# tiangexiang/OccNeRF

Hardware: AMD Instinct MI355X
Metric: rays/sec at 512x512x128spp, random-init ckpt (higher is better)
Workload: dtype f32; 1 GPU; BASELINE configs[1]: free-view frame, 512x512 image, 128 samples/ray, non-rigid motion on, seeded random-init checkpoint; synthetic SMPL-like body and camera; 183784 rays hit the body bbox (ray_mask); H2D of the ray batch and the prior and D2H of [R,5] inside the step; the frame's rays sharded over the ranks; samples whose motion-weight sum is exactly 0 are dropped after the warp (bit-identical pi; rays_per_frame=183784, samples_per_ray=128, skip_empty_samples=True, dedup_repeated_samples=False, knn_center_cache=True, warp_bone_culling=True, world_size_formed=1

## Files before the change

include/occnerf_hip.h:

```cpp
#ifndef OCCNERF_HIP_H
#define OCCNERF_HIP_H

#include <stdint.h>

#ifdef __cplusplus
extern "C" {
#endif

#define OCCNERF_ABI_VERSION 5

int occnerf_abi_version(void);
const char *occnerf_last_error(void);

int occnerf_experiment_knob(const char *name, int value);


int occnerf_grid_encode_forward(const float *inputs, const float *embeddings,
                                const int32_t *offsets, float *outputs, uint32_t B, uint32_t D,
                                uint32_t C, uint32_t L, float S, uint32_t H, float *dy_dx,
                                uint32_t gridtype, int align_corners, uint32_t interp,
                                void *stream);

int occnerf_grid_encode_backward(const float *grad, const float *inputs, const float *embeddings,
                                 const int32_t *offsets, float *grad_embeddings, uint32_t B,
// ... 289 lines not shown
                         const double *h_dist, int32_t win_y, int32_t win_x, int32_t win_h, int32_t win_w,
                         uint8_t *out_image, uint8_t *out_mask, void *stream);

int occnerf_resize_frame(const uint8_t *image, const uint8_t *mask, int32_t H, int32_t W, int32_t h, int32_t w,
                         const int32_t *x_off_lanczos, const float *x_w_lanczos, const int32_t *y_off_lanczos,
                         const float *y_w_lanczos, const int32_t *x_off_bilinear, const float *x_w_bilinear,
                         const int32_t *y_off_bilinear, const float *y_w_bilinear, const int32_t *h_x_off_lanczos,
                         const int32_t *h_y_off_lanczos, const int32_t *h_x_off_bilinear, const int32_t *h_y_off_bilinear,
                         const float *h_bgcolor, double *img64, double *alpha64, void *stream);

int occnerf_patch_batch_f64(const double *img64, const double *alpha64, const float *rays8, const uint8_t *box_mask,
                            int32_t H, int32_t W, int32_t n_patches, int32_t size, const double *h_u, double subject_ratio,
                            const float *h_bgcolor, int32_t *row_counts, float *rays, float *near, float *far,
                            float *target_rgbs, float *target_patches, uint8_t *patch_masks, int32_t *patch_div_indices,
                            int32_t *xy_min, int32_t *pix_of_row, int32_t *row_of_pix, int32_t *n_rows, void *stream);
int occnerf_whole_frame_gather_f64(const double *img64, const double *alpha64, const float *rays8, const uint8_t *box_mask,
                                   int32_t H, int32_t W, const float *h_bgcolor, const int32_t *row_start, int32_t R,
                                   int64_t *ray_index, float *rays, float *near, float *far, float *target_rgbs,
                                   double *ray_alpha, uint8_t *truth_u8, float *gt_vis, float *gt_alpha, void *stream);

#define OCCNERF_FRAME_METRICS_RECORD 14
int64_t occnerf_frame_metrics_workspace_bytes(int32_t N, int32_t H, int32_t W);
int occnerf_frame_metrics(const uint8_t *pred, const uint8_t *truth, const float *alpha, const uint8_t *body,
                          const float *gt_vis_alpha, const float *gt_alpha, int32_t N, int32_t H, int32_t W,
                          double data_range, double *record, double *ssim_map, void *workspace, void *stream);

int32_t occnerf_progress_tile_blocks(int32_t height, int32_t width);
int occnerf_progress_tile(const float *rgb, const int64_t *ray_index, int64_t R, int32_t height, int32_t width,
                          const float *h_bgcolor01, const double *h_bgcolor255, const uint8_t *truth_u8, uint8_t *mosaic,
                          int32_t mosaic_rows, int32_t mosaic_cols, int32_t tile_x, int32_t tile_y, int32_t *partial,
                          int32_t *off_bg, void *stream);


int occnerf_mesh_count(const float *field, int32_t nx, int32_t ny, int32_t nz, float level, int32_t *row_count,
                       void *stream);
int occnerf_mesh_emit(const float *field, int32_t nx, int32_t ny, int32_t nz, float level, const int64_t *row_start,
                      int64_t T, int64_t *tri_keys, void *stream);
int occnerf_mesh_vertices(const int64_t *keys, int64_t V, const float *field, int32_t nx, int32_t ny, int32_t nz,
                          float level, const double *h_bbox_min, double h, float *pos, void *stream);

int occnerf_mesh_pose(const float *x_c, int64_t V, const float *Rs, const float *Ts, const float *vol, int32_t nb, int32_t G,
                      const float *h_bbox_min, const float *h_bbox_scale, int32_t candidates, int32_t max_iter, double tol,
                      float *p_out, uint8_t *flag, uint8_t *iters, float *resid, void *stream);


int occnerf_mesh_project(const float *pos, int64_t V, const double *h_K, const double *h_E, int32_t *xy, double *z,
                         uint8_t *vflag, void *stream);
int occnerf_mesh_raster(const int32_t *faces, int64_t T, int64_t V, const int32_t *xy, const double *z, const uint8_t *vflag,
                        int32_t H, int32_t W, uint64_t *keys, int32_t *wide_list, int32_t *counts, void *stream);
int occnerf_mesh_resolve(const uint64_t *keys, const int32_t *faces, int64_t T, int64_t V, const int32_t *xy, const double *z,
                         const uint8_t *vflag, const uint8_t *colors, const uint8_t *h_bgcolor, int32_t H, int32_t W,
                         uint8_t *cover, int32_t *tri, float *depth, uint8_t *rgb, int32_t *counts, void *stream);

#ifdef __cplusplus
}
#endif
#endif
```

occnerf_amd/_lib.py:

```python
import ctypes as C
import os

_HERE = os.path.dirname(os.path.abspath(__file__))
LIB_PATH = os.environ.get('OCCNERF_HIP_LIB') or os.path.join(_HERE, 'liboccnerf_hip.so')

ABI_VERSION = 5

_vp, _i32, _i64, _u32, _f32 = C.c_void_p, C.c_int32, C.c_int64, C.c_uint32, C.c_float

SIGNATURES = {
    'occnerf_abi_version': (C.c_int, []),
    'occnerf_last_error': (C.c_char_p, []),
    'occnerf_experiment_knob': (C.c_int, [C.c_char_p, C.c_int]),
    'occnerf_grid_encode_forward': (C.c_int, [_vp, _vp, _vp, _vp, _u32, _u32, _u32, _u32, _f32, _u32,
                                               _vp, _u32, C.c_int, _u32, _vp]),
    'occnerf_grid_encode_backward': (C.c_int, [_vp, _vp, _vp, _vp, _vp, _u32, _u32, _u32, _u32, _f32,
                                                _u32, _vp, _vp, _u32, C.c_int, _u32, _vp]),
    'occnerf_grid_grad_runs': (C.c_int, [_vp, _vp, _i64, _u32, _u32, _u32, _vp, _vp]),
    'occnerf_grid_encode_forward_h': (C.c_int, [_vp, _vp, _vp, _vp, _vp, _u32, _u32, _u32, _u32, _f32, _u32,
                                                 _vp, _u32, C.c_int, _u32, _vp]),
    'occnerf_grid_encode_backward_h': (C.c_int, [_vp, _vp, _vp, _vp, _vp, _vp, _u32, _u32, _u32, _u32, _f32,
                                                  _u32, _vp, _vp, _u32, C.c_int, _u32, _vp, _i64, _vp]),
    'occnerf_grid_encode_forward_f16': (C.c_int, [_vp, _vp, _vp, _vp, _u32, _u32, _u32, _u32, _f32, _u32,
                                                   _vp, _u32, C.c_int, _u32, _vp]),
# ... 67 lines not shown
    'occnerf_canonical_mlp_bf16x3': (C.c_int, [_vp, _i64, _vp, _vp, _vp, _i32, _vp]),
    'occnerf_canonical_mlp_pack_f16': (C.c_int, [_vp, _vp, _vp]),
    'occnerf_canonical_mlp_f16x3': (C.c_int, [_vp, _vp, _i64, _vp, _vp, _vp, _vp, _vp, _vp]),
    'occnerf_nonrigid_pack_f16': (C.c_int, [_vp, _vp, _vp]),
    'occnerf_nonrigid_f16x3': (C.c_int, [_vp, _i64, _vp, _vp, _vp, _vp, _vp, _vp, _vp, _vp, _vp, _vp, _vp]),
    'occnerf_canonical_mlp_bf16x3_rows': (C.c_int, [_vp, _vp, _i64, _vp, _vp, _vp, _vp, _i32, _vp]),
    'occnerf_composite': (C.c_int, [_vp, _vp, _vp, _vp, _vp, _i64, _i32, _vp, _vp, _vp, _vp, _vp, _vp, _vp]),
    'occnerf_linear_pack': (C.c_int, [_vp, _vp, _i32, _i32, _vp, _i32, _vp, _i32, _i32, _vp, _vp, _vp, _vp]),
    'occnerf_linear_forward': (C.c_int, [_vp, _i64, _i32, _vp, _i64, _i32, _vp, _vp, _i32, _vp, _i64, _vp, _i64, _i32,
                                          _i32, _vp, _i32, _i64, _i64, _i32, _i32, _vp]),
    'occnerf_linear_wgrad_slices': (_i32, [_i64]),
    'occnerf_linear_wgrad': (C.c_int, [_vp, _i64, _i32, _vp, _i64, _i32, _i64, _i32, _vp, _vp, _vp]),
    'occnerf_linear_wgrad_reduce': (C.c_int, [_vp, _vp, _i32, _i32, _i32, _vp, _vp, _vp, _i32, _vp, _i32, _vp]),
    'occnerf_composite_backward': (C.c_int, [_vp, _vp, _vp, _vp, _vp, _i64, _i32, _vp, _vp, _vp, _vp, _vp, _vp]),
    'occnerf_warp_backward_slices': (_i32, [_i64]),
    'occnerf_warp_backward': (C.c_int, [_vp, _i64, _i32, _vp, _vp, _vp, _vp, _vp, _i32, _i32, _vp, _vp, _vp, _vp, _vp]),
    'occnerf_agg_weights': (C.c_int, [_vp, _vp, _i64, _i32, _vp, _vp, _vp]),
    'occnerf_pose_motion_bases': (C.c_int, [_vp, _vp, _vp, _i32, _vp, _vp, _vp, _vp, _vp, _vp]),
    'occnerf_pose_motion_bases_backward': (C.c_int, [_vp, _vp, _vp, _vp, _vp, _vp, _vp, _vp, _vp, _vp, _vp]),
    'occnerf_prior_softmax': (C.c_int, [_vp, _vp, _i32, _i64, _vp, _vp]),
    'occnerf_pack_rays': (C.c_int, [_vp, _vp, _vp, _vp, _i64, _vp, _vp]),
    'occnerf_assemble_image': (C.c_int, [_vp, _vp, _vp, _i64, _i32, _i32, _vp, _vp, _vp, _vp]),
    'occnerf_convt3d_col2im': (C.c_int, [_vp, _vp, _i32, _i32, _i32, _i32, _vp, _vp]),
    'occnerf_convt3d_im2col': (C.c_int, [_vp, _i32, _i32, _i32, _i32, _vp, _vp]),
    'occnerf_adam_table_row_bytes': (_i32, []),
    'occnerf_adam_step': (C.c_int, [_vp, _i32, _vp, _i32, _i32] + [C.c_double] * 4 + [_vp, _vp]),
    'occnerf_lpips_packed_floats': (_i64, []),
    'occnerf_lpips_workspace_floats': (_i64, [_i32, _i32, _i32]),
    'occnerf_lpips_pack': (C.c_int, [_vp, _vp, _vp, _vp, _vp, _vp, _vp]),
    'occnerf_lpips_forward': (C.c_int, [_vp, _vp, _vp, _i32, _i32, _i32, _i32, _vp, _vp, _vp, _vp]),
    'occnerf_lpips_backward': (C.c_int, [_vp, _vp, _i32, _i32, _i32, _i32, _vp, _vp, _vp, _vp]),
    'occnerf_patch_assemble': (C.c_int, [_vp, _vp, _i64, _i32, _i32, _vp, _vp, _vp]),
    'occnerf_patch_assemble_backward': (C.c_int, [_vp, _vp, _i64, _vp, _vp]),
    'occnerf_patch_batch_max_patches': (_i32, []),
    'occnerf_patch_batch': (C.c_int, [_vp, _vp, _vp, _vp, _i32, _i32, _i32, _i32, _vp, C.c_double, _vp] + [_vp] * 12 + [_vp]),
    'occnerf_whole_frame_count': (C.c_int, [_vp, _i32, _i32, _vp, _vp]),
    'occnerf_whole_frame_gather': (C.c_int, [_vp, _vp, _vp, _vp, _i32, _i32, _vp, _vp, _i32] + [_vp] * 9 + [_vp]),
    'occnerf_view_frame_gather': (C.c_int, [_vp, _vp, _i32, _i32, _vp, _i32, _vp, _vp, _vp, _vp, _vp]),
    'occnerf_undistort_u8': (C.c_int, [_vp, _vp, _i32, _i32, _vp, _vp, _i32, _i32, _i32, _i32, _vp, _vp, _vp]),
    'occnerf_resize_frame': (C.c_int, [_vp, _vp, _i32, _i32, _i32, _i32] + [_vp] * 8 + [_vp] * 4 + [_vp, _vp, _vp, _vp]),
    'occnerf_patch_batch_f64': (C.c_int, [_vp, _vp, _vp, _vp, _i32, _i32, _i32, _i32, _vp, C.c_double, _vp] + [_vp] * 12 + [_vp]),
    'occnerf_whole_frame_gather_f64': (C.c_int, [_vp, _vp, _vp, _vp, _i32, _i32, _vp, _vp, _i32] + [_vp] * 9 + [_vp]),
    'occnerf_frame_metrics_workspace_bytes': (_i64, [_i32, _i32, _i32]),
    'occnerf_frame_metrics': (C.c_int, [_vp, _vp, _vp, _vp, _vp, _vp, _i32, _i32, _i32, C.c_double, _vp, _vp, _vp, _vp]),
    'occnerf_progress_tile_blocks': (_i32, [_i32, _i32]),
    'occnerf_progress_tile': (C.c_int, [_vp, _vp, _i64, _i32, _i32, _vp, _vp, _vp, _vp, _i32, _i32, _i32, _i32, _vp, _vp, _vp]),
    'occnerf_mesh_count': (C.c_int, [_vp, _i32, _i32, _i32, _f32, _vp, _vp]),
    'occnerf_mesh_emit': (C.c_int, [_vp, _i32, _i32, _i32, _f32, _vp, _i64, _vp, _vp]),
    'occnerf_mesh_vertices': (C.c_int, [_vp, _i64, _vp, _i32, _i32, _i32, _f32, _vp, C.c_double, _vp, _vp]),
    'occnerf_mesh_pose': (C.c_int, [_vp, _i64, _vp, _vp, _vp, _i32, _i32, _vp, _vp, _i32, _i32, C.c_double, _vp, _vp, _vp, _vp, _vp]),
    'occnerf_mesh_project': (C.c_int, [_vp, _i64, _vp, _vp, _vp, _vp, _vp, _vp]),
    'occnerf_mesh_raster': (C.c_int, [_vp, _i64, _i64, _vp, _vp, _vp, _i32, _i32, _vp, _vp, _vp, _vp]),
    'occnerf_mesh_resolve': (C.c_int, [_vp, _vp, _i64, _i64, _vp, _vp, _vp, _vp, _vp, _i32, _i32, _vp, _vp, _vp, _vp, _vp, _vp]),
}

_lib = None


def lib():
    global _lib
    if _lib is None:
        if not os.path.exists(LIB_PATH):
            raise ImportError(
                f'{LIB_PATH} not found: the gfx950 kernels are not built. Run '
                '`python -c "import __graft_entry__ as g; g.build()"` (or `make -C '
                'occnerf_amd/csrc`). There is no CPU fallback for this path.')
        import torch
        handle = C.CDLL(LIB_PATH)
        for name, (res, args) in SIGNATURES.items():
            fn = getattr(handle, name)
            fn.restype, fn.argtypes = res, args
        if handle.occnerf_abi_version() != ABI_VERSION:
            raise ImportError(f'liboccnerf_hip.so: ABI version {handle.occnerf_abi_version()}, this binding was written '
                              f'for {ABI_VERSION} (include/occnerf_hip.h OCCNERF_ABI_VERSION): rebuild the library')
        _lib = handle
    return _lib


def check(rc, what):
    if rc != 0:
        msg = lib().occnerf_last_error().decode(errors='replace')
        raise RuntimeError(f'{what} failed ({rc}): {msg}')
```

occnerf_amd/csrc/compact.hip:

```cpp
#include "common.h"

#include <hipcub/hipcub.hpp>

namespace occ {

struct LivePredicate {
    const float *mask;
    __device__ bool operator()(const int &i) const { return mask[i] != 0.0f; }
};

__global__ void scatter_raw_kernel(const float *__restrict__ raw_c, const int32_t *__restrict__ rows,
                                   const int32_t *__restrict__ n_dev, float *__restrict__ raw_full) {
    const int64_t m = (int64_t)blockIdx.x * blockDim.x + threadIdx.x;
    if (m >= (int64_t)*n_dev) return;
    const int64_t n = rows[m];
#pragma unroll
    for (int c = 0; c < 5; c++) raw_full[n * 5 + c] = raw_c[m * 5 + c];
}

struct RepeatFlag {
    const uint32_t *keys;
    int64_t stride;
    int K;
    const int32_t *rows;
// ... 240 lines not shown
        hipLaunchKernelGGL(unique_remap_kernel, dim3((unsigned)((scan_cap + 255) / 256)), dim3(256), 0, st, scan, n_scan_dev,
                           rep);
    return check_launch("unique_heads");
}

OCC_API int occnerf_scatter_raw_heads(const float *raw_h, const float *raw_c, const int32_t *rows, const int32_t *n_dev,
                                      const int32_t *scanA, const int32_t *scanB, int64_t N_max, float *raw_full,
                                      void *stream) {
    using namespace occ;
    if (N_max <= 0) return 0;
    OCC_REQUIRE(raw_h && raw_c && rows && n_dev && raw_full, "scatter_raw_heads: null argument");
    const int64_t blocks = (N_max + 255) / 256;
    OCC_REQUIRE(blocks < (1ll << 31), "scatter_raw_heads: N too large");
    hipLaunchKernelGGL(scatter_raw_heads_kernel, dim3((unsigned)blocks), dim3(256), 0, as_stream(stream), raw_h, raw_c,
                       rows, n_dev, scanA, scanB, raw_full);
    return check_launch("scatter_raw_heads");
}

OCC_API int64_t occnerf_live_rows_temp_bytes(int64_t N) {
    using namespace occ;
    if (N <= 0 || N >= (1ll << 31)) return 0;
    size_t bytes = 0;
    hipcub::CountingInputIterator<int> it(0);
    if (hipcub::DeviceSelect::If(nullptr, bytes, it, (int *)nullptr, (int *)nullptr, (int)N, LivePredicate{nullptr},
                                 (hipStream_t)0) != hipSuccess)
        return -1;
    return (int64_t)bytes;
}

OCC_API int occnerf_live_rows(const float *mask, int64_t N, int32_t *rows, int32_t *count, void *temp,
                              int64_t temp_bytes, void *stream) {
    using namespace occ;
    OCC_REQUIRE(mask && rows && count && temp, "live_rows: null argument");
    OCC_REQUIRE(N > 0 && N < (1ll << 31), "live_rows: N=%lld out of range", (long long)N);
    size_t bytes = (size_t)temp_bytes;
    hipcub::CountingInputIterator<int> it(0);
    const hipError_t e = hipcub::DeviceSelect::If(temp, bytes, it, rows, count, (int)N, LivePredicate{mask},
                                                  as_stream(stream));
    OCC_REQUIRE(e == hipSuccess, "live_rows: %s", hipGetErrorString(e));
    return check_launch("live_rows");
}

OCC_API int occnerf_scatter_raw(const float *raw_c, const int32_t *rows, const int32_t *n_dev, int64_t N_max,
                                float *raw_full, void *stream) {
    using namespace occ;
    if (N_max <= 0) return 0;
    OCC_REQUIRE(raw_c && rows && n_dev && raw_full, "scatter_raw: null argument");
    const int64_t blocks = (N_max + 255) / 256;
    OCC_REQUIRE(blocks < (1ll << 31), "scatter_raw: N too large");
    hipLaunchKernelGGL(scatter_raw_kernel, dim3((unsigned)blocks), dim3(256), 0, as_stream(stream), raw_c, rows, n_dev,
                       raw_full);
    return check_launch("scatter_raw");
}
```

occnerf_amd/network.py:

```python
import os

import numpy as np
import torch
import torch.nn as nn

from . import geometry, ops
from .canonical_mlp import CanonicalMLP
from .config import get_cfg
from .rayorder import ray_patch_order
from .modules import (BodyPoseRefiner, MotionBasisComputer, MotionWeightVolumeDecoder,
                      NonRigidMotionMLP, hann_window_weights)


class _Replica(nn.Module):

    def __init__(self, module):
        super().__init__()
        self.module = module

    def forward(self, *a, **k):
        return self.module(*a, **k)


def _load_smpl(cfg):
# ... 175 lines not shown
        dec_mod = self.mweight_vol_decoder
        enc = self.cnl_mlp.module.encoder
        srcs = list(dec_mod.parameters()) + [self.point_dist, self.point_base, enc.embeddings]
        key = tuple((t.data_ptr(), t._version) for t in srcs)
        if self._wconst is not None and self._wconst['key'] == key:
            return self._wconst
        with torch.no_grad():
            dec = dec_mod.decoder.forward_gemm(dec_mod.const_embedding[None])[0].contiguous()
            table = self._point_stage(self._context())
        self._wconst = {'key': key, 'dec': dec, 'table': table}
        return self._wconst

    def _point_pack(self, wc):
        srcs = [self.point_counter, self.point_base]
        key = (wc['table'].data_ptr(),) + tuple((t.data_ptr(), t._version) for t in srcs)
        if wc.get('pack_key') != key:
            ctx = self._context()
            wc['pack'] = ops.point_pack(self.point_base.detach(), ctx['normals'], ctx['unit'],
                                        self.point_counter.detach(), wc['table'])
            wc['pack_key'] = key
        return wc['pack']

    def _point_stage(self, ctx):
        enc = self.cnl_mlp.module.encoder
        pc = self.point_cloud.detach().float().contiguous()
        base = self.point_base.detach()
        kidx = ops.knn_small(pc, base, 3)
        knn_base, sdf = ops.point_sdf(pc, base, ctx['normals'], ctx['unit'], kidx)
        table = ops.point_table(knn_base, sdf, pc, ctx['bound32'], ctx['two_bound32'],
                                enc.embeddings.detach(), enc.offsets, enc.log2_per_level_scale,
                                enc.base_resolution)
        return table

    def _stage_features(self, rays8, z, xyz, mask, pk, cond, hann, table, pack, center=None):
        cfg, ctx = self.cfg, self._context()
        S = int(cfg.N_samples)
        enc = self.cnl_mlp.module.encoder
        rows, count = ops.live_rows(mask)
        self.last_live_count = count
        dedup = bool(cfg.get('dedup_repeated_samples', True))
        scan_a = scan_b = mrows = mcount = None
        frows, fcount, kmask = rows, count, mask
        if not cfg.ignore_non_rigid_motions:
            if pk['nr_bf16'] is not None:
                ops.nonrigid_bf16x3_rows(xyz, rows, count, cond, hann, pk['nr_w0'], pk['nr_b0'], pk['nr'], pk['nr_bf16'],
                                         domain_flag=pk['domain_flag'])
            else:
                ops.nonrigid_rows(xyz, rows, count, cond, hann, pk['nr_w0'], pk['nr_b0'], pk['nr'])
        if dedup:
            scan_a, frows, fcount, kmask = ops.repeat_heads(xyz, 3, count, rows=rows,
                                                            want_mask=not cfg.get('knn_query_list', True))
            if cfg.get('dedup_global_positions', False):
                frows, fcount = ops.unique_heads(xyz, 3, frows, fcount, scan=scan_a, scan_count=count)
        self.last_head_counts = (fcount, None)
        if cfg.get('knn_query_list', True):
            knn = ops.msknn_clustered(xyz, rays8.shape[0], S, ctx['clusters'], ctx['seed'], rows=frows, count=fcount, center=center)
        else:
            knn = ops.msknn_clustered(xyz, rays8.shape[0], S, ctx['clusters'], ctx['seed'], mask=kmask, center=center)
        if center is not None and len(center) > 3 and center[3] != self._center_stamp(table):
            raise RuntimeError('stale kNN centre: its cached feature row was computed from another table / counter / embedding '
                               'version than this frame\'s (ops.sample_features freshness contract)')
        mlp_in, raw_c, _ = ops.sample_features(
            xyz, knn, self.point_base.detach(), ctx['normals'], ctx['unit'],
            self.point_counter.detach(), table, ctx['bound32'], ctx['two_bound32'],
            enc.embeddings.detach(), enc.offsets, enc.log2_per_level_scale, enc.base_resolution,
            rows=frows, count=fcount, pack=pack, center=None if center is None else center[0],
            center_agg=None if center is None else center[2])
        del knn
        if dedup:
            scan_b, mrows, mcount, _ = ops.repeat_heads(mlp_in, 68, fcount)
            if cfg.get('dedup_global', True):
                mrows, mcount = ops.unique_heads(mlp_in, 68, mrows, mcount, scan=scan_b, scan_count=fcount)
            self.last_head_counts = (fcount, mcount)
        return {'dedup': dedup, 'rays8': rays8, 'z': z, 'mask': mask, 'rows': rows, 'count': count, 'mlp_in': mlp_in,
                'raw_c': raw_c, 'scan_a': scan_a, 'scan_b': scan_b, 'mrows': mrows, 'mcount': mcount, 'cnl': pk['cnl'],
                'cnl_bf16': pk['cnl_bf16'], 'domain_flag': pk['domain_flag'], 'N': xyz.shape[0]}

    @staticmethod
    def _stage_mlp_composite(st, bgcolor, out, out_rows):
        dev, N = st['mlp_in'].device, st['N']

        def mlp(raw_out, count, in_rows=None):
            if st['cnl_bf16'] is not None:
                ops.canonical_mlp_bf16x3(st['mlp_in'], st['cnl'], st['cnl_bf16'], raw_out, count=count, in_rows=in_rows,
                                         domain_flag=st['domain_flag'])
            else:
                ops.canonical_mlp(st['mlp_in'], st['cnl'], raw_out, count=count, in_rows=in_rows)
        if st['dedup']:
            raw_h = torch.empty(st['mlp_in'].shape[0], 5, device=dev)
            mlp(raw_h, st['mcount'], st['mrows'])
            raw = ops.scatter_raw_heads(raw_h, st['raw_c'], st['rows'], st['count'], st['scan_a'], st['scan_b'],
                                        torch.zeros(N, 5, device=dev))
        else:
            mlp(st['raw_c'], st['count'])
            raw = ops.scatter_raw(st['raw_c'], st['rows'], st['count'], torch.zeros(N, 5, device=dev))
        st['mlp_in'] = None
        return ops.composite(raw, st['mask'], st['z'], st['rays8'], bgcolor, out=out, out_rows=out_rows)[:3]

    def _nonrigid_f16_pack(self):
        pk = self._packed_weights()
        if pk.get('nr_f16_train') is None:
            nr_lin = [m for m in self.non_rigid_mlp.module.block_mlps if isinstance(m, nn.Linear)]
            pk['nr_f16_train'] = pk['nr_bf16'] if (pk['nr_bf16'] is not None and pk['nr_bf16'].dtype == torch.float16) else \
                ops.nonrigid_pack_f16([m.weight.detach() for m in nr_lin])
        return pk['nr_f16_train']

    def _knn_center_lists(self, cond, hann):
        ctx, pk = self._context(), self._packed_weights()
        c = torch.zeros(64, 3, device=self.point_base.device)
        if not self.cfg.ignore_non_rigid_motions:
            c = ops.nonrigid(c, cond, hann, pk['nr_w0'], pk['nr_b0'], pk['nr'], direct=True)
        return ops.knn_center(c[0].contiguous(), ctx['points'], ctx['index_map'], ctx['scale_begin'])

    def _knn_center(self, cond, hann, table, pack):
        ctx, pk = self._context(), self._packed_weights()
        c = torch.zeros(64, 3, device=self.point_base.device)
        if not self.cfg.ignore_non_rigid_motions:
            c = ops.nonrigid(c, cond, hann, pk['nr_w0'], pk['nr_b0'], pk['nr'], direct=True)
        center, idx = ops.knn_center(c[0].contiguous(), ctx['points'], ctx['index_map'], ctx['scale_begin'])
        enc = self.cnl_mlp.module.encoder
        row, _, enc_in = ops.sample_features(
            c[:8].contiguous(), idx[None].expand(8, -1, -1).contiguous(), self.point_base.detach(), ctx['normals'], ctx['unit'],
            self.point_counter.detach(), table, ctx['bound32'], ctx['two_bound32'], enc.embeddings.detach(), enc.offsets,
            enc.log2_per_level_scale, enc.base_resolution, pack=pack, want_enc_in=True)
        return center, idx, ops.center_row(row[0], enc_in[0]), self._center_stamp(table)

    def _center_stamp(self, table):
        return (table.data_ptr(), table._version, self.point_counter._version, self.cnl_mlp.module.encoder.embeddings._version)

    def _render_rays(self, rays8, Rs, Ts, vol, bbox_min, bbox_scale, bgcolor, cond, hann,
                     table, t_rand=None, out=None, out_rows=None, pack=None, boxes=None, center=None):
        cfg, ctx = self.cfg, self._context()
        S = int(cfg.N_samples)
        enc = self.cnl_mlp.module.encoder
        t_vals = torch.linspace(0., 1., steps=S, device=rays8.device)
        z, xyz, mask, _ = ops.sample_warp(rays8, S, t_vals, Rs, Ts, vol, bbox_min, bbox_scale,
                                          t_rand=t_rand, boxes=boxes)
        pk = self._packed_weights()
        N = xyz.shape[0]
        if cfg.get('skip_empty_samples', True) and cfg.get('knn_culling', True):
            st = self._stage_features(rays8, z, xyz, mask, pk, cond, hann, table, pack, center)
            return self._stage_mlp_composite(st, bgcolor, out, out_rows)

        if not cfg.ignore_non_rigid_motions:
            if pk['nr_bf16'] is not None:
                ops.nonrigid_bf16x3(xyz, cond, hann, pk['nr_w0'], pk['nr_b0'], pk['nr'], pk['nr_bf16'], out=xyz, domain_flag=pk['domain_flag'])
            else:
# ... 264 lines not shown
```

occnerf_amd/ops.py:

```python
import ctypes as C

import numpy as np
import torch

from . import _lib

_f32p = C.POINTER(C.c_float)


def _chk(t, dtype, name):
    if not torch.is_tensor(t):
        raise RuntimeError(f'{name} must be a tensor')
    if not t.is_cuda:
        raise RuntimeError(f'{name} must be a CUDA(HIP) tensor; there is no CPU path')
    if not t.is_contiguous():
        raise RuntimeError(f'{name} must be a contiguous tensor')
    if t.dtype != dtype:
        raise RuntimeError(f'{name} must be {dtype}, got {t.dtype}')
    return t.data_ptr()


def _guard_dev(dev):
    if torch.device(dev).type != 'cuda':
        raise RuntimeError(f'tensors are on {dev}: this path runs on a GPU only, there is no CPU path')
# ... 211 lines not shown
    return packed


def nonrigid(xyz, cond, hann, W0, b0, packed, out=None, direct=False):
    out = torch.empty_like(xyz) if out is None else out
    _kh, ph = _host_f32(hann, 6)
    fn = _lib.lib().occnerf_nonrigid_direct if direct else _lib.lib().occnerf_nonrigid
    with _guard(xyz):
        rc = fn(
            _chk(xyz, torch.float32, 'xyz'), xyz.shape[0], _chk(cond, torch.float32, 'cond'), ph,
            _chk(W0, torch.float32, 'W0'), _chk(b0, torch.float32, 'b0'),
            _chk(packed, torch.float32, 'packed'), _chk(out, torch.float32, 'xyz_out'), _stream(xyz))
    _lib.check(rc, 'nonrigid')
    return out


def nonrigid_rows(xyz, rows, count, cond, hann, W0, b0, packed):
    _kh, ph = _host_f32(hann, 6)
    with _guard(xyz):
        rc = _lib.lib().occnerf_nonrigid_rows(
            _chk(xyz, torch.float32, 'xyz'), rows.shape[0], _chk(rows, torch.int32, 'rows'),
            _chk(count, torch.int32, 'count'), _chk(cond, torch.float32, 'cond'), ph,
            _chk(W0, torch.float32, 'W0'), _chk(b0, torch.float32, 'b0'), _chk(packed, torch.float32, 'packed'),
            _stream(xyz))
    _lib.check(rc, 'nonrigid_rows')
    return xyz


def live_rows(mask):
    N = mask.shape[0]
    dev = mask.device
    nbytes = int(_lib.lib().occnerf_live_rows_temp_bytes(N))
    if nbytes < 0:
        raise RuntimeError('live_rows: temp size query failed')
    temp = torch.empty(max(nbytes, 16), device=dev, dtype=torch.uint8)
    rows = torch.empty(N, device=dev, dtype=torch.int32)
    count = torch.empty(1, device=dev, dtype=torch.int32)
    with _guard(mask):
        rc = _lib.lib().occnerf_live_rows(_chk(mask, torch.float32, 'mask'), N, rows.data_ptr(), count.data_ptr(),
                                          temp.data_ptr(), nbytes, _stream(mask))
    _lib.check(rc, 'live_rows')
    return rows, count


def scatter_raw(raw_c, rows, count, raw_full):
    with _guard(raw_c):
        rc = _lib.lib().occnerf_scatter_raw(_chk(raw_c, torch.float32, 'raw_c'), _chk(rows, torch.int32, 'rows'),
                                            _chk(count, torch.int32, 'count'), rows.shape[0],
                                            _chk(raw_full, torch.float32, 'raw_full'), _stream(raw_c))
    _lib.check(rc, 'scatter_raw')
    return raw_full


def repeat_heads(keys, key_cols, count, rows=None, want_mask=False):
    dev = keys.device
    if keys.dim() != 2 or not keys.is_contiguous() or keys.element_size() != 4:
        raise RuntimeError('repeat_heads: keys must be a contiguous [M, C] tensor of 4-byte elements')
    cap = keys.shape[0] if rows is None else rows.shape[0]
    scan = torch.empty(cap, device=dev, dtype=torch.int32)
    heads = torch.empty(cap, device=dev, dtype=torch.int32)
    head_count = torch.empty(1, device=dev, dtype=torch.int32)
    head_mask = torch.zeros(keys.shape[0], device=dev, dtype=torch.float32) if want_mask else None
    if cap == 0:
        head_count.zero_()
        return scan, heads, head_count, head_mask
    nbytes = int(_lib.lib().occnerf_repeat_heads_temp_bytes(cap))
    if nbytes < 0:
        raise RuntimeError('repeat_heads: temp size query failed')
    temp = torch.empty(max(nbytes, 16), device=dev, dtype=torch.uint8)
    with _guard_dev(dev):
        rc = _lib.lib().occnerf_repeat_heads(
            keys.data_ptr(), keys.shape[1], int(key_cols), _opt(rows, torch.int32, 'rows'),
            _chk(count, torch.int32, 'count'), cap, scan.data_ptr(), heads.data_ptr(), head_count.data_ptr(),
            None if head_mask is None else head_mask.data_ptr(), temp.data_ptr(), nbytes, _stream(keys))
    _lib.check(rc, 'repeat_heads')
    return scan, heads, head_count, head_mask


def unique_heads(keys, key_cols, heads, count, scan=None, scan_count=None):
    dev = keys.device
    if keys.dim() != 2 or not keys.is_contiguous() or keys.element_size() != 4:
        raise RuntimeError('unique_heads: keys must be a contiguous [M, C] tensor of 4-byte elements')
    cap = keys.shape[0] if heads is None else heads.shape[0]
    heads_out = torch.empty(cap, device=dev, dtype=torch.int32)
    count_out = torch.empty(1, device=dev, dtype=torch.int32)
    if cap == 0:
        count_out.zero_()
        return heads_out, count_out
    nbytes = int(_lib.lib().occnerf_unique_heads_temp_bytes(cap))
    if nbytes <= 0:
        raise RuntimeError('unique_heads: temp size query failed')
    temp = torch.empty(nbytes, device=dev, dtype=torch.uint8)
    with _guard_dev(dev):
        rc = _lib.lib().occnerf_unique_heads(
            keys.data_ptr(), keys.shape[1], int(key_cols), _opt(heads, torch.int32, 'heads'),
            _chk(count, torch.int32, 'count'), cap, heads_out.data_ptr(), count_out.data_ptr(),
            _opt(scan, torch.int32, 'scan'), _opt(scan_count, torch.int32, 'scan_count'),
            0 if scan is None else scan.shape[0], temp.data_ptr(), nbytes, _stream(keys))
    _lib.check(rc, 'unique_heads')
    return heads_out, count_out


def scatter_raw_heads(raw_h, raw_c, rows, count, scan_a, scan_b, raw_full):
    with _guard(raw_c):
        rc = _lib.lib().occnerf_scatter_raw_heads(
            _chk(raw_h, torch.float32, 'raw_h'), _chk(raw_c, torch.float32, 'raw_c'), _chk(rows, torch.int32, 'rows'),
# ... 134 lines not shown
    return out


def point_sdf(point_cloud, point_base, normals, unit, kidx):
    P = point_cloud.shape[0]
    kb = torch.empty(P, 3, device=point_cloud.device, dtype=torch.float64)
    dist = torch.empty(P, device=point_cloud.device, dtype=torch.float32)
    with _guard(point_cloud):
        rc = _lib.lib().occnerf_point_sdf(
            _chk(point_cloud, torch.float32, 'point_cloud'), _chk(point_base, torch.float32, 'point_base'),
            _chk(normals, torch.float64, 'normals'), _chk(unit, torch.float64, 'unit_normals'),
            _chk(kidx, torch.int32, 'kidx'), P, kb.data_ptr(), dist.data_ptr(), _stream(point_cloud))
    _lib.check(rc, 'point_sdf')
    return kb, dist


def table_stride():
    return int(_lib.lib().occnerf_point_table_stride())


def point_table(knn_base, sdf, learnable, bound32, two_bound32, embeddings, offsets, S, H):
    P = knn_base.shape[0]
    table = torch.empty(P, table_stride(), device=knn_base.device, dtype=torch.float32)
    with _guard(knn_base):
        rc = _lib.lib().occnerf_point_table(
            _chk(knn_base, torch.float64, 'knn_base'), _chk(sdf, torch.float32, 'point_sdf'),
            _chk(learnable, torch.float32, 'learnable'), P, float(bound32), float(two_bound32),
            _chk(embeddings, torch.float32, 'embeddings'), _chk(offsets, torch.int32, 'offsets'),
            _host_offsets(offsets), int(offsets.shape[0] - 1), float(S), int(H), table.data_ptr(),
            _stream(knn_base))
    _lib.check(rc, 'point_table')
    return table


def point_pack(point_base, normals, unit, counter, table):
    P, dev = point_base.shape[0], point_base.device
    geo = torch.empty(P, 16, device=dev, dtype=torch.float32)
    tail = torch.empty(P, 4, device=dev, dtype=torch.float32)
    with _guard_dev(dev):
        rc = _lib.lib().occnerf_point_pack(
            _chk(point_base, torch.float32, 'point_base'), _chk(normals, torch.float64, 'normals'),
            _chk(unit, torch.float64, 'unit_normals'), _chk(counter, torch.float32, 'counter'),
            _chk(table, torch.float32, 'table'), P, geo.data_ptr(), tail.data_ptr(), _stream(point_base))
    _lib.check(rc, 'point_pack')
    return geo, tail


def center_row(mlp_in_row, enc_in_row):
    return torch.cat([mlp_in_row[:36], enc_in_row[:4], mlp_in_row[36:68]]).contiguous()


def sample_features(xyz, knn_idxs, point_base, normals, unit, counter, table, bound32, two_bound32,
                    embeddings, offsets, S, H, raw=None, want_enc_in=False, geo_idxs=None,
                    att_in=None, rows=None, count=None, pack=None, center=None, center_agg=None):
    N = xyz.shape[0] if rows is None else rows.shape[0]
    dev = xyz.device
    if (pack is None and N > 0 and knn_idxs.shape[1] == 4 and geo_idxs is None and att_in is None
            and counter is not None and table.dim() == 2 and table.shape[1] == table_stride()):
        pack = point_pack(point_base, normals, unit, counter, table)
    geo, tail = pack if pack is not None else (None, None)
    if table.dim() != 2 or table.shape[1] != table_stride():
        raise RuntimeError(f'sample_features: table must be [P,{table_stride()}] (ops.point_table), got {tuple(table.shape)}')
    mlp_in = torch.empty(N, 68, device=dev, dtype=torch.float32)
    raw = torch.empty(N, 5, device=dev, dtype=torch.float32) if raw is None else raw
    enc_in = torch.empty(N, 4, device=dev, dtype=torch.float32) if want_enc_in else None
    with _guard_dev(dev):
        rc = _lib.lib().occnerf_sample_features_centered(
            _chk(xyz, torch.float32, 'xyz'), N, _chk(knn_idxs, torch.int32, 'knn_idxs'),
            int(knn_idxs.shape[1]), _chk(point_base, torch.float32, 'point_base'),
            _chk(normals, torch.float64, 'normals'), _chk(unit, torch.float64, 'unit_normals'),
            _opt(counter, torch.float32, 'counter'), _chk(table, torch.float32, 'table'),
            float(bound32), float(two_bound32), _chk(embeddings, torch.float32, 'embeddings'),
            _chk(offsets, torch.int32, 'offsets'), _host_offsets(offsets), int(offsets.shape[0] - 1),
            float(S), int(H), _opt(geo_idxs, torch.int32, 'geo_idxs'), _opt(att_in, torch.float32, 'att_in'),
            _opt(rows, torch.int32, 'rows'), _opt(count, torch.int32, 'count'),
            _opt(geo, torch.float32, 'point_geo'), _opt(tail, torch.float32, 'point_tail'),
            0 if geo is None else int(geo.shape[0]),
            _opt(center, torch.float32, 'center'), _opt(center_agg, torch.float32, 'center_agg'),
            mlp_in.data_ptr(), _chk(raw, torch.float32, 'raw'),
            None if enc_in is None else enc_in.data_ptr(), _stream(xyz))
    _lib.check(rc, 'sample_features')
    return mlp_in, raw, enc_in


def canonical_mlp_pack(weights, biases):
    dev = weights[0].device
    n = _lib.lib().occnerf_canonical_mlp_packed_floats()
    packed = torch.zeros(n, device=dev, dtype=torch.float32)
    with _guard_dev(dev):
        rc = _lib.lib().occnerf_canonical_mlp_pack(_ptr_table(weights, 'W'), _ptr_table(biases, 'b'),
                                                   packed.data_ptr(), _stream(packed))
    _lib.check(rc, 'canonical_mlp_pack')
    return packed


def canonical_mlp(mlp_in, packed, raw, direct=False, count=None, in_rows=None):
    if in_rows is not None:
        with _guard(mlp_in):
            rc = _lib.lib().occnerf_canonical_mlp_rows(
                _chk(mlp_in, torch.float32, 'mlp_in'), _chk(in_rows, torch.int32, 'in_rows'), in_rows.shape[0],
                _chk(count, torch.int32, 'count'), _chk(packed, torch.float32, 'packed'),
                _chk(raw, torch.float32, 'raw'), _stream(mlp_in))
        _lib.check(rc, 'canonical_mlp_rows')
        return raw
    if count is not None:
        with _guard(mlp_in):
            rc = _lib.lib().occnerf_canonical_mlp_counted(
                _chk(mlp_in, torch.float32, 'mlp_in'), mlp_in.shape[0], _chk(count, torch.int32, 'count'),
                _chk(packed, torch.float32, 'packed'), _chk(raw, torch.float32, 'raw'), _stream(mlp_in))
        _lib.check(rc, 'canonical_mlp_counted')
        return raw
    fn = _lib.lib().occnerf_canonical_mlp_direct if direct else _lib.lib().occnerf_canonical_mlp
    with _guard(mlp_in):
        rc = fn(_chk(mlp_in, torch.float32, 'mlp_in'), mlp_in.shape[0], _chk(packed, torch.float32, 'packed'),
                _chk(raw, torch.float32, 'raw'), _stream(mlp_in))
    _lib.check(rc, 'canonical_mlp')
    return raw


def trunks_pack_bf16(weights, out=None):
    dev = weights[0].device
    if out is None:
        out = torch.zeros(_lib.lib().occnerf_trunks_packed_bytes() // 2, device=dev, dtype=torch.bfloat16)
    with _guard_dev(dev):
        rc = _lib.lib().occnerf_trunks_pack_bf16(_ptr_table(weights[:9], 'W'), out.data_ptr(), _stream(out))
    _lib.check(rc, 'trunks_pack_bf16')
    return out


def trunks_forward_bf16(agg, var, enc, packed_f32, packed_bf16):
    M, dev, bf = agg.shape[0], agg.device, torch.bfloat16
    X0 = torch.empty(M, 96, device=dev, dtype=bf)
# ... 724 lines not shown
```

Measured before the change: 1.229 million rays/s.

## Route samples matching the cached KNN centre row to a shared MLP input row

Adds a classify kernel that, for samples inside the cached KNN-centre sphere, recomputes the 10-neighbour aggregate. It flags samples whose features bit-match the precomputed centre row and writes their signed distance directly. A hipcub select then compacts the remaining samples, so the KNN query and feature kernels run only on those. Flagged samples are mapped through in_rows to a single appended centre row in the MLP input buffer. This saves KNN and feature work for centre-region samples, at the cost of an extra classify pass, a device select, a temp allocation and a scatter-merge of distances.

```diff
diff --git a/include/occnerf_hip.h b/include/occnerf_hip.h
--- a/include/occnerf_hip.h
+++ b/include/occnerf_hip.h
@@ -365,6 +365,17 @@
                          const uint8_t *vflag, const uint8_t *colors, const uint8_t *h_bgcolor, int32_t H, int32_t W,
                          uint8_t *cover, int32_t *tri, float *depth, uint8_t *rgb, int32_t *counts, void *stream);
 
+int occnerf_center_classify(const float *xyz, const int32_t *rows, const int32_t *n_dev, int64_t N_max,
+                            const float *point_geo, int32_t P, const float *center, const int32_t *center_idx,
+                            const float *center_agg, float bound, float two_bound, uint8_t *flag, float *raw_c,
+                            void *stream);
+int64_t occnerf_center_split_temp_bytes(int64_t N_max);
+int occnerf_center_split(const uint8_t *flag, const int32_t *rows, const int32_t *n_dev, int64_t N_max,
+                         int32_t centre_row, int32_t *keep, int32_t *rows2, int32_t *count2, int32_t *in_rows,
+                         int32_t *taken, void *temp, int64_t temp_bytes, void *stream);
+int occnerf_center_merge_dist(const float *raw2, const int32_t *keep, const int32_t *n2_dev, int64_t N_max, float *raw_c,
+                              void *stream);
+
 #ifdef __cplusplus
 }
 #endif
diff --git a/occnerf_amd/_lib.py b/occnerf_amd/_lib.py
--- a/occnerf_amd/_lib.py
+++ b/occnerf_amd/_lib.py
@@ -143,6 +143,10 @@
     'occnerf_mesh_project': (C.c_int, [_vp, _i64, _vp, _vp, _vp, _vp, _vp, _vp]),
     'occnerf_mesh_raster': (C.c_int, [_vp, _i64, _i64, _vp, _vp, _vp, _i32, _i32, _vp, _vp, _vp, _vp]),
     'occnerf_mesh_resolve': (C.c_int, [_vp, _vp, _i64, _i64, _vp, _vp, _vp, _vp, _vp, _i32, _i32, _vp, _vp, _vp, _vp, _vp, _vp]),
+    'occnerf_center_classify': (C.c_int, [_vp, _vp, _vp, _i64, _vp, _i32, _vp, _vp, _vp, _f32, _f32, _vp, _vp, _vp]),
+    'occnerf_center_split_temp_bytes': (_i64, [_i64]),
+    'occnerf_center_split': (C.c_int, [_vp, _vp, _vp, _i64, _i32, _vp, _vp, _vp, _vp, _vp, _vp, _i64, _vp]),
+    'occnerf_center_merge_dist': (C.c_int, [_vp, _vp, _vp, _i64, _vp, _vp]),
 }
 
 _lib = None
diff --git a/occnerf_amd/csrc/center.hip b/occnerf_amd/csrc/center.hip
--- /dev/null
+++ b/occnerf_amd/csrc/center.hip
@@ -0,0 +1,125 @@
+#include "common.h"
+
+namespace occ {
+
+constexpr int kKnn = 10;
+
+__device__ __forceinline__ double cos3_unit(const float (&a)[3], const double (&un)[3]) {
+    float na = norm3(a[0], a[1], a[2]);
+    na = na < 1e-8f ? 1e-8f : na;
+    const double t0 = __dmul_rn((double)__fdiv_rn(a[0], na), un[0]);
+    const double t1 = __dmul_rn((double)__fdiv_rn(a[1], na), un[1]);
+    const double t2 = __dmul_rn((double)__fdiv_rn(a[2], na), un[2]);
+    return __dadd_rn(__dadd_rn(t0, t1), t2);
+}
+
+struct GeoRec {
+    float base[3], pad;
+    double normal[3], unit[3];
+};
+static_assert(sizeof(GeoRec) == 64, "GeoRec is the 64-byte record of occnerf_point_pack");
+
+constexpr int kClassifyBlock = 256;
+
+__global__ __launch_bounds__(kClassifyBlock) void center_classify_kernel(
+    const float *__restrict__ xyz, const int32_t *__restrict__ rows, const int32_t *__restrict__ n_dev,
+    const GeoRec *__restrict__ geo, int P, const float *__restrict__ center, const int32_t *__restrict__ center_idx,
+    const float *__restrict__ center_agg, float bound, float two_bound, uint8_t *__restrict__ flag,
+    float *__restrict__ raw_c) {
+    const int64_t o = (int64_t)blockIdx.x * blockDim.x + threadIdx.x;
+    const int64_t n = (int64_t)*n_dev;
+    if ((int64_t)blockIdx.x * blockDim.x >= n) return;
+    const bool live = o < n;
+    const float ccx = center[0], ccy = center[1], ccz = center[2], cr2 = center[3];
+    float p[3] = {0.f, 0.f, 0.f};
+    bool inside = false;
+    if (live) {
+        const int64_t i = rows[o];
+        struct __attribute__((packed, aligned(4))) F3 { float v[3]; };
+        const F3 pq = *reinterpret_cast<const F3 *>(xyz + i * 3);
+        p[0] = pq.v[0], p[1] = pq.v[1], p[2] = pq.v[2];
+        const float dx = p[0] - ccx, dy = p[1] - ccy, dz = p[2] - ccz;
+        inside = __builtin_fmaf(dz, dz, __builtin_fmaf(dy, dy, dx * dx)) < cr2;
+    }
+    bool take = false;
+    if (inside) {
+        int neg = 0;
+        float dsum = 0.0f;
+        double num[3] = {0.0, 0.0, 0.0}, den = 0.0;
+#pragma unroll
+        for (int j = 0; j < kKnn; j++) {
+            int id = center_idx[j];
+            id = id < 0 ? 0 : (id >= P ? P - 1 : id);
+            const GeoRec r = geo[id];
+            float dir[3];
+#pragma unroll
+            for (int c = 0; c < 3; c++) dir[c] = __fsub_rn(p[c], r.base[c]);
+            double dot = __dadd_rn(0.0, __dmul_rn((double)dir[0], r.normal[0]));
+            dot = __dadd_rn(dot, __dmul_rn((double)dir[1], r.normal[1]));
+            dot = __dadd_rn(dot, __dmul_rn((double)dir[2], r.normal[2]));
+            neg += dot < 0.0;
+            dsum = __fadd_rn(dsum, norm3(dir[0], dir[1], dir[2]));
+            if (j < 3) {
+                const double att = fabs(cos3_unit(dir, r.unit));
+#pragma unroll
+                for (int c = 0; c < 3; c++) {
+                    const float pn = __fdiv_rn(__fadd_rn(r.base[c], bound), two_bound);
+                    num[c] = __dadd_rn(num[c], __dmul_rn(att, (double)pn));
+                }
+                den = __dadd_rn(den, att);
+            }
+        }
+        float dist = __fdiv_rn(dsum, (float)kKnn);
+        if (2 * neg > kKnn) dist = -dist;
+        float nd = __fdiv_rn(__fadd_rn(dist, 0.2f), 0.5f);
+        nd = nd < 0.0f ? 0.0f : (nd > 1.0f ? 1.0f : nd);
+        float x[4];
+#pragma unroll
+        for (int c = 0; c < 3; c++) x[c] = (float)__ddiv_rn(num[c], den);
+        x[3] = nd;
+        take = inside && __float_as_uint(x[0]) == __float_as_uint(center_agg[36]) &&
+               __float_as_uint(x[1]) == __float_as_uint(center_agg[37]) &&
+               __float_as_uint(x[2]) == __float_as_uint(center_agg[38]) &&
+               __float_as_uint(x[3]) == __float_as_uint(center_agg[39]);
+        if (take) raw_c[o * 5 + 4] = dist;
+    }
+    if (live) flag[o] = take ? 1 : 0;
+}
+
+__global__ void center_merge_dist_kernel(const float *__restrict__ raw2, const int32_t *__restrict__ keep,
+                                         const int32_t *__restrict__ n2_dev, float *__restrict__ raw_c) {
+    const int64_t o2 = (int64_t)blockIdx.x * blockDim.x + threadIdx.x;
+    if (o2 >= (int64_t)*n2_dev) return;
+    raw_c[(int64_t)keep[o2] * 5 + 4] = raw2[o2 * 5 + 4];
+}
+
+}
+
+OCC_API int occnerf_center_classify(const float *xyz, const int32_t *rows, const int32_t *n_dev, int64_t N_max,
+                                    const float *point_geo, int32_t P, const float *center, const int32_t *center_idx,
+                                    const float *center_agg, float bound, float two_bound, uint8_t *flag, float *raw_c,
+                                    void *stream) {
+    using namespace occ;
+    if (N_max <= 0) return 0;
+    OCC_REQUIRE(xyz && rows && n_dev && point_geo && center && center_idx && center_agg && flag && raw_c,
+                "center_classify: null argument");
+    OCC_REQUIRE(P > 0, "center_classify: P=%d rows of packed point records", P);
+    const int64_t blocks = (N_max + kClassifyBlock - 1) / kClassifyBlock;
+    OCC_REQUIRE(blocks < (1ll << 31), "center_classify: N too large");
+    hipLaunchKernelGGL(center_classify_kernel, dim3((unsigned)blocks), dim3(kClassifyBlock), 0, as_stream(stream), xyz, rows, n_dev,
+                       reinterpret_cast<const GeoRec *>(point_geo), (int)P, center, center_idx, center_agg, bound, two_bound,
+                       flag, raw_c);
+    return check_launch("center_classify");
+}
+
+OCC_API int occnerf_center_merge_dist(const float *raw2, const int32_t *keep, const int32_t *n2_dev, int64_t N_max,
+                                      float *raw_c, void *stream) {
+    using namespace occ;
+    if (N_max <= 0) return 0;
+    OCC_REQUIRE(raw2 && keep && n2_dev && raw_c, "center_merge_dist: null argument");
+    const int64_t blocks = (N_max + 255) / 256;
+    OCC_REQUIRE(blocks < (1ll << 31), "center_merge_dist: N too large");
+    hipLaunchKernelGGL(center_merge_dist_kernel, dim3((unsigned)blocks), dim3(256), 0, as_stream(stream), raw2, keep,
+                       n2_dev, raw_c);
+    return check_launch("center_merge_dist");
+}
diff --git a/occnerf_amd/csrc/compact.hip b/occnerf_amd/csrc/compact.hip
--- a/occnerf_amd/csrc/compact.hip
+++ b/occnerf_amd/csrc/compact.hip
@@ -316,3 +316,56 @@
                        raw_full);
     return check_launch("scatter_raw");
 }
+
+namespace occ {
+
+struct KeepPredicate {
+    const uint8_t *flag;
+    const int32_t *n_dev;
+    __device__ bool operator()(const int &o) const { return o < *n_dev && flag[o] == 0; }
+};
+
+__global__ void center_split_kernel(const uint8_t *__restrict__ flag, const int32_t *__restrict__ rows,
+                                    const int32_t *__restrict__ n_dev, const int32_t *__restrict__ keep,
+                                    const int32_t *__restrict__ count2, int32_t centre_row, int32_t *__restrict__ rows2,
+                                    int32_t *__restrict__ in_rows, int32_t *__restrict__ taken) {
+    const int64_t m = (int64_t)blockIdx.x * blockDim.x + threadIdx.x;
+    const int64_t n = *n_dev, n2 = *count2;
+    if (m == 0) *taken = (int32_t)(n - n2);
+    if (m < n && flag[m] != 0) in_rows[m] = centre_row;
+    if (m < n2) {
+        const int32_t o = keep[m];
+        rows2[m] = rows[o];
+        in_rows[o] = (int32_t)m;
+    }
+}
+
+}
+
+OCC_API int64_t occnerf_center_split_temp_bytes(int64_t N) {
+    using namespace occ;
+    if (N <= 0 || N >= (1ll << 31)) return 0;
+    size_t bytes = 0;
+    hipcub::CountingInputIterator<int> it(0);
+    if (hipcub::DeviceSelect::If(nullptr, bytes, it, (int *)nullptr, (int *)nullptr, (int)N, KeepPredicate{nullptr, nullptr},
+                                 (hipStream_t)0) != hipSuccess)
+        return -1;
+    return (int64_t)bytes;
+}
+
+OCC_API int occnerf_center_split(const uint8_t *flag, const int32_t *rows, const int32_t *n_dev, int64_t N_max,
+                                 int32_t centre_row, int32_t *keep, int32_t *rows2, int32_t *count2, int32_t *in_rows,
+                                 int32_t *taken, void *temp, int64_t temp_bytes, void *stream) {
+    using namespace occ;
+    OCC_REQUIRE(flag && rows && n_dev && keep && rows2 && count2 && in_rows && taken && temp, "center_split: null argument");
+    OCC_REQUIRE(N_max > 0 && N_max < (1ll << 31), "center_split: N=%lld out of range", (long long)N_max);
+    size_t bytes = (size_t)temp_bytes;
+    hipcub::CountingInputIterator<int> it(0);
+    const hipError_t e = hipcub::DeviceSelect::If(temp, bytes, it, keep, count2, (int)N_max, KeepPredicate{flag, n_dev},
+                                                  as_stream(stream));
+    OCC_REQUIRE(e == hipSuccess, "center_split: %s", hipGetErrorString(e));
+    const int64_t blocks = (N_max + 255) / 256;
+    hipLaunchKernelGGL(center_split_kernel, dim3((unsigned)blocks), dim3(256), 0, as_stream(stream), flag, rows, n_dev, keep,
+                       count2, centre_row, rows2, in_rows, taken);
+    return check_launch("center_split");
+}
diff --git a/occnerf_amd/network.py b/occnerf_amd/network.py
--- a/occnerf_amd/network.py
+++ b/occnerf_amd/network.py
@@ -251,6 +251,22 @@
                                                             want_mask=not cfg.get('knn_query_list', True))
             if cfg.get('dedup_global_positions', False):
                 frows, fcount = ops.unique_heads(xyz, 3, frows, fcount, scan=scan_a, scan_count=count)
+        split = None
+        self.last_center_taken = None
+        want = cfg.get('center_split', 'auto')
+        if want == 'auto':
+            want = pk['nr_bf16'] is None or bool(cfg.ignore_non_rigid_motions)
+        if not dedup and center is not None and len(center) > 2 and pack is not None and want and cfg.get('knn_query_list', True):
+            M = rows.shape[0]
+            raw_c = torch.empty(M, 5, device=xyz.device)
+            flag = ops.center_classify(xyz, rows, count, pack[0], center[0], center[1], center[2], ctx['bound32'],
+                                       ctx['two_bound32'], raw_c)
+            keep, frows, fcount, in_rows, taken = ops.center_split(flag, rows, count, M)
+            mlp_buf = torch.empty(M + 1, 68, device=xyz.device)
+            mlp_buf[M, :36] = center[2][:36]
+            mlp_buf[M, 36:] = center[2][40:72]
+            split = {'keep': keep, 'count2': fcount, 'in_rows': in_rows, 'raw_c': raw_c, 'mlp_buf': mlp_buf}
+            self.last_center_taken = taken
         self.last_head_counts = (fcount, None)
         if cfg.get('knn_query_list', True):
             knn = ops.msknn_clustered(xyz, rays8.shape[0], S, ctx['clusters'], ctx['seed'], rows=frows, count=fcount, center=center)
@@ -264,15 +280,19 @@
             self.point_counter.detach(), table, ctx['bound32'], ctx['two_bound32'],
             enc.embeddings.detach(), enc.offsets, enc.log2_per_level_scale, enc.base_resolution,
             rows=frows, count=fcount, pack=pack, center=None if center is None else center[0],
-            center_agg=None if center is None else center[2])
+            center_agg=None if center is None else center[2], mlp_in_out=None if split is None else split['mlp_buf'])
         del knn
+        in_rows = None
+        if split is not None:
+            raw_c = ops.center_merge_dist(raw_c, split['keep'], split['count2'], split['raw_c'])
+            in_rows = split['in_rows']
         if dedup:
             scan_b, mrows, mcount, _ = ops.repeat_heads(mlp_in, 68, fcount)
             if cfg.get('dedup_global', True):
                 mrows, mcount = ops.unique_heads(mlp_in, 68, mrows, mcount, scan=scan_b, scan_count=fcount)
             self.last_head_counts = (fcount, mcount)
         return {'dedup': dedup, 'rays8': rays8, 'z': z, 'mask': mask, 'rows': rows, 'count': count, 'mlp_in': mlp_in,
-                'raw_c': raw_c, 'scan_a': scan_a, 'scan_b': scan_b, 'mrows': mrows, 'mcount': mcount, 'cnl': pk['cnl'],
+                'raw_c': raw_c, 'in_rows': in_rows, 'scan_a': scan_a, 'scan_b': scan_b, 'mrows': mrows, 'mcount': mcount, 'cnl': pk['cnl'],
                 'cnl_bf16': pk['cnl_bf16'], 'domain_flag': pk['domain_flag'], 'N': xyz.shape[0]}
 
     @staticmethod
@@ -291,7 +311,7 @@
             raw = ops.scatter_raw_heads(raw_h, st['raw_c'], st['rows'], st['count'], st['scan_a'], st['scan_b'],
                                         torch.zeros(N, 5, device=dev))
         else:
-            mlp(st['raw_c'], st['count'])
+            mlp(st['raw_c'], st['count'], st['in_rows'])
             raw = ops.scatter_raw(st['raw_c'], st['rows'], st['count'], torch.zeros(N, 5, device=dev))
         st['mlp_in'] = None
         return ops.composite(raw, st['mask'], st['z'], st['rays8'], bgcolor, out=out, out_rows=out_rows)[:3]
diff --git a/occnerf_amd/ops.py b/occnerf_amd/ops.py
--- a/occnerf_amd/ops.py
+++ b/occnerf_amd/ops.py
@@ -287,6 +287,58 @@
     return raw_full
 
 
+def center_classify(xyz, rows, count, geo, center, center_idx, center_agg, bound32, two_bound32, raw_c, flag=None):
+    M = rows.shape[0]
+    if flag is None:
+        flag = torch.empty(M, device=xyz.device, dtype=torch.uint8)
+    if flag.shape[0] < M or raw_c.shape[0] < M:
+        raise RuntimeError('center_classify: flag and raw_c need a row per list entry')
+    if center_idx.numel() < 10 or center_agg.numel() < 72 or center.numel() < 4:
+        raise RuntimeError('center_classify: center[4], center_idx[>= 10] and center_agg[72] (ops.knn_center, ops.center_row)')
+    with _guard(xyz):
+        rc = _lib.lib().occnerf_center_classify(
+            _chk(xyz, torch.float32, 'xyz'), _chk(rows, torch.int32, 'rows'), _chk(count, torch.int32, 'count'), M,
+            _chk(geo, torch.float32, 'point_geo'), int(geo.shape[0]), _chk(center, torch.float32, 'center'),
+            _chk(center_idx, torch.int32, 'center_idx'), _chk(center_agg, torch.float32, 'center_agg'),
+            float(bound32), float(two_bound32), _chk(flag, torch.uint8, 'flag'), _chk(raw_c, torch.float32, 'raw_c'),
+            _stream(xyz))
+    _lib.check(rc, 'center_classify')
+    return flag
+
+
+def center_split(flag, rows, count, centre_row):
+    M, dev = rows.shape[0], rows.device
+    keep = torch.empty(M, device=dev, dtype=torch.int32)
+    rows2 = torch.empty(M, device=dev, dtype=torch.int32)
+    in_rows = torch.empty(M, device=dev, dtype=torch.int32)
+    count2 = torch.empty(1, device=dev, dtype=torch.int32)
+    taken = torch.empty(1, device=dev, dtype=torch.int32)
+    if M == 0:
+        count2.zero_()
+        taken.zero_()
+        return keep, rows2, count2, in_rows, taken
+    nbytes = int(_lib.lib().occnerf_center_split_temp_bytes(M))
+    if nbytes < 0:
+        raise RuntimeError('center_split: temp size query failed')
+    temp = torch.empty(max(nbytes, 16), device=dev, dtype=torch.uint8)
+    with _guard(rows):
+        rc = _lib.lib().occnerf_center_split(
+            _chk(flag, torch.uint8, 'flag'), _chk(rows, torch.int32, 'rows'), _chk(count, torch.int32, 'count'), M,
+            int(centre_row), keep.data_ptr(), rows2.data_ptr(), count2.data_ptr(), in_rows.data_ptr(), taken.data_ptr(),
+            temp.data_ptr(), nbytes, _stream(rows))
+    _lib.check(rc, 'center_split')
+    return keep, rows2, count2, in_rows, taken
+
+
+def center_merge_dist(raw2, keep, count2, raw_c):
+    with _guard(raw2):
+        rc = _lib.lib().occnerf_center_merge_dist(
+            _chk(raw2, torch.float32, 'raw2'), _chk(keep, torch.int32, 'keep'), _chk(count2, torch.int32, 'count2'),
+            keep.shape[0], _chk(raw_c, torch.float32, 'raw_c'), _stream(raw2))
+    _lib.check(rc, 'center_merge_dist')
+    return raw_c
+
+
 def repeat_heads(keys, key_cols, count, rows=None, want_mask=False):
     dev = keys.device
     if keys.dim() != 2 or not keys.is_contiguous() or keys.element_size() != 4:
@@ -527,7 +579,7 @@
 
 def sample_features(xyz, knn_idxs, point_base, normals, unit, counter, table, bound32, two_bound32,
                     embeddings, offsets, S, H, raw=None, want_enc_in=False, geo_idxs=None,
-                    att_in=None, rows=None, count=None, pack=None, center=None, center_agg=None):
+                    att_in=None, rows=None, count=None, pack=None, center=None, center_agg=None, mlp_in_out=None):
     N = xyz.shape[0] if rows is None else rows.shape[0]
     dev = xyz.device
     if (pack is None and N > 0 and knn_idxs.shape[1] == 4 and geo_idxs is None and att_in is None
@@ -536,7 +588,12 @@
     geo, tail = pack if pack is not None else (None, None)
     if table.dim() != 2 or table.shape[1] != table_stride():
         raise RuntimeError(f'sample_features: table must be [P,{table_stride()}] (ops.point_table), got {tuple(table.shape)}')
-    mlp_in = torch.empty(N, 68, device=dev, dtype=torch.float32)
+    if mlp_in_out is None:
+        mlp_in = torch.empty(N, 68, device=dev, dtype=torch.float32)
+    else:
+        mlp_in = mlp_in_out
+        if mlp_in.dim() != 2 or mlp_in.shape[0] < N or mlp_in.shape[1] != 68:
+            raise RuntimeError(f'sample_features: mlp_in_out must be [>= {N}, 68], got {tuple(mlp_in.shape)}')
     raw = torch.empty(N, 5, device=dev, dtype=torch.float32) if raw is None else raw
     enc_in = torch.empty(N, 4, device=dev, dtype=torch.float32) if want_enc_in else None
     with _guard_dev(dev):
@@ -552,7 +609,7 @@
             _opt(geo, torch.float32, 'point_geo'), _opt(tail, torch.float32, 'point_tail'),
             0 if geo is None else int(geo.shape[0]),
             _opt(center, torch.float32, 'center'), _opt(center_agg, torch.float32, 'center_agg'),
-            mlp_in.data_ptr(), _chk(raw, torch.float32, 'raw'),
+            _chk(mlp_in, torch.float32, 'mlp_in'), _chk(raw, torch.float32, 'raw'),
             None if enc_in is None else enc_in.data_ptr(), _stream(xyz))
     _lib.check(rc, 'sample_features')
     return mlp_in, raw, enc_in
```

New measurement: 1.246 million rays/s (median of 6 runs). 1.01x the previous value.
